# yjhuangcd/rule-guided-music

Hardware: AMD Instinct MI355X
Metric: denoising steps/sec (whole node), DiTRotary_XL_8 4x128x16 (higher is better)
Workload: dtype f32 via bf16x3_presplit split (3 bf16 MFMA per product, fp32 accumulate); 1 GPU; C2 unconditional DDIM-50 (eta=1), DiTRotary_XL_8, batch 16 per GPU, latent 4x128x16; batch_per_gpu=16, weights=synthetic random-init (rgm.synth seed 1; adaLN/final layers re-randomised), timing=one timed region of 255 steps

## Files before the change

### include/rgm.h

```cpp
#ifndef RGM_H
#define RGM_H

#include <stddef.h>
#include <stdint.h>

#ifdef __cplusplus
extern "C" {
#endif

typedef enum {
  RGM_OK = 0,
  RGM_ERR_INVALID = -1,
  RGM_ERR_HIP = -2,
  RGM_ERR_WORKSPACE = -3,
  RGM_ERR_STATE = -4
} rgm_status;

int rgm_version(void);
const char* rgm_last_error(void);

typedef struct rgm_dit rgm_dit;

typedef struct {
  int32_t depth;
  int32_t hidden;
  int32_t heads;
  int32_t patch;
  int32_t in_ch;
  int32_t out_ch;
  int32_t width;
  int32_t n_embed;
  int32_t kind;
  int32_t n_out;
  int32_t max_tokens;
} rgm_dit_cfg;

int rgm_dit_create(const rgm_dit_cfg* cfg, rgm_dit** out);
void rgm_dit_destroy(rgm_dit* h);
int rgm_dit_set_param(rgm_dit* h, const char* key, const void* dptr, const int64_t* shape, int ndim);
int rgm_dit_missing_params(rgm_dit* h);
size_t rgm_dit_workspace_bytes(const rgm_dit* h, int N, int H);
int rgm_dit_forward(rgm_dit* h, const float* x, const int64_t* t, const int32_t* y, float* eps,
                    int N, int H, void* ws, size_t ws_bytes, void* stream);
int rgm_dit_cond_rows(rgm_dit* h, const int64_t* t, const int32_t* y, int U, int H, float* rows, void* ws, size_t ws_bytes, void* stream);
int rgm_dit_forward_cond(rgm_dit* h, const float* x, const float* rows, const int32_t* idx, int U, float* eps,
                         int N, int H, void* ws, size_t ws_bytes, void* stream);
int rgm_dit_classify(rgm_dit* h, const float* x, const int64_t* t, float* logits, float* key_out,
                     int N, int H, void* ws, size_t ws_bytes, void* stream);

int rgm_gemm(const float* A, int lda, const float* B, int ldb, float* C, int ldc, int M, int N, int K,
             const float* bias, int act, float alpha, const float* gate, int gate_ld, int rows_per_gate,
             const float* res, int ldres, void* stream);
int rgm_layernorm_modulate(const float* x, float* out, int M, int D, float eps, const float* weight,
                           const float* bias, const float* shift, const float* scale, int mod_ld,
                           int rows_per_batch, void* stream);
int rgm_adaln_stream(const float* cs, const float* W, const float* bias, float* mod, int N, int D, int L, void* stream);
int rgm_rotary_attention(const float* qkv, float* o, const float* cos_tab, const float* sin_tab,
                         int N, int T, int heads, int hd, int rot_half, void* stream);
int rgm_rotary_attention_lse(const float* qkv, float* o, float* lse, const float* cos_tab, const float* sin_tab,
                             int N, int T, int heads, int hd, int rot_half, void* stream);

int rgm_set_gemm_precision(int prec);
int rgm_get_gemm_precision(void);
int rgm_split_dtype(void);
int rgm_split_rows(const float* x, float* out, int64_t rows, int K, void* stream);
int rgm_gemm_split(const float* A_split, const float* B_split, float* C, int M, int N, int K, const float* bias,
                   int act, int tile, int out_split, void* stream);
int rgm_split_rows_ld(const float* x, int ld_in, float* out, int ld_out, int64_t rows, int K, void* stream);
int rgm_gemm_split_ld(const float* A_split, int lda, const float* B_split, int ldb, float* C, int ldc, int M, int N, int K,
                      const float* bias, int act, int tile, int out_split, void* stream);
int rgm_set_big_tiles(int mode, int min_tiles);
int rgm_set_fuse_reduce_ln(int on);
long long rgm_fused_reduce_ln_launches(void);
int rgm_set_adaln_overlap(int on);
int rgm_set_gn_fuse(int mode, int* prev);
long long rgm_gn_fused_launches(void);
long long rgm_gn_fallback_tiles(int reset);
int rgm_set_dit_halves(int min_batch, int* prev);
int rgm_set_attn_pairs(int on);
int rgm_set_attn_stream(int on);
size_t rgm_gemm_scratch_bytes(int M, int N);
int rgm_gemm_split_ws(const float* A_split, const float* B_split, float* C, int M, int N, int K, const float* bias, int act,
                      int tile, int out_split, void* ws, size_t ws_bytes, void* stream);
int rgm_gemm_split_epi(const float* A_split, int lda, const float* B_split, int ldb, float* C, int ldc, int M, int N, int K,
                       const float* bias, int act, float alpha, const float* gate, int gate_ld, int rows_per_gate,
                       const float* res, int ldres, int tile, int out_split, void* ws, size_t ws_bytes, void* stream);
int rgm_gemm_tile(const float* A, int lda, const float* B, int ldb, float* C, int ldc, int M, int N, int K,
                  const float* bias, int act, int tile, void* stream);

int rgm_randn(float* out, int64_t n, uint64_t seed, uint64_t offset, void* stream);
int rgm_ddpm_step(const float* x, const float* eps, const float* grad, const float* noise, const int64_t* t,
                  const float* const* tables_host, int clip_denoised, int t_end, float* sample, float* pred_xstart,
                  float* g_out, int N, int E, void* stream);
int rgm_ddpm_step_learned(const float* x, const float* eps, const float* var_values, const float* min_log_tab,
                          const float* max_log_tab, const float* grad, const float* noise, const int64_t* t,
                          const float* const* tables_host, int clip_denoised, int t_end, float* sample, float* pred_xstart, int N,
                          int E, void* stream);
int rgm_ddpm_step_learned_g(const float* x, const float* eps, const float* var_values, const float* min_log_tab,
                            const float* max_log_tab, const float* grad, const float* noise, const int64_t* t,
                            const float* const* tables_host, int clip_denoised, int t_end, float* sample, float* pred_xstart,
                            float* g_elem, int N, int E, void* stream);
int rgm_ddim_step(const float* x, const float* eps, const float* grad, const float* noise, const int64_t* t,
                  const float* const* tables_host, int clip_denoised, int t_end, float eta, float* sample,
                  float* pred_xstart, float* g_out, int N, int E, void* stream);
int rgm_dpmpp_step(const float* x, const float* eps, const float* grad, const float* x0_prev, const float* noise, const int64_t* t,
                   const float* const* tables_host, const float* const* dpm_tables_host, int num_timesteps, int order,
                   int clip_denoised, int t_end, float* sample, float* pred_xstart, float* g_out, int N, int E, void* stream);
int rgm_ddim_reverse_step(const float* x, const float* eps, const int64_t* t, const float* const* tables_host, int num_timesteps,
                          int clip_denoised, float* sample, float* pred_xstart, int N, int E, void* stream);
int64_t rgm_vb_terms_partials(int N, int E);
int rgm_vb_terms(const float* x_start, const float* x_t, const float* eps, const float* noise, const int64_t* t,
                 const float* const* tables_host, const float* post_logvar_tab, const float* var_values, const float* min_log_tab,
                 const float* max_log_tab, const float* model_mean, const float* model_xstart, int clip_denoised, double* partials,
                 float* vb, float* xstart_mse, float* eps_mse, float* pred_xstart, int N, int E, void* stream);
int rgm_prior_bpd(const float* x_start, float sqrt_alphas_cumprod_T, float log_one_minus_alphas_cumprod_T, double* partials, float* out,
                  int N, int E, void* stream);
int rgm_scg_candidates(const float* mean, const float* g, const float* noise, float* cand, int n, int B, int E,
                       void* stream);
int rgm_xstart_from_eps(const float* x, const float* eps, const int64_t* t, const float* const* tables_host,
                        float out_scale, float* out, int N, int E, void* stream);
int rgm_edit_replace_eps(const float* x, const float* eps, const float* gt, const float* mask, const int64_t* t,
                         const float* const* tables_host, int clip_denoised, float* eps_out, int N, int E, void* stream);
int rgm_scg_select(const float* cand, const float* total_logp, float* out, int64_t* max_ind, int n, int B, int E,
                   void* stream);
int rgm_scg_rebuild(const float* mean, const float* g, const int64_t* max_ind, uint64_t seed, uint64_t base, float* out,
                    int B, int E, int H, int W, int seg_rows, void* stream);
int rgm_scg_rebuild_g(const float* mean, const float* g_elem, const int64_t* max_ind, uint64_t seed, uint64_t base, float* out,
                      int B, int E, int H, int W, int seg_rows, void* stream);

typedef struct rgm_vae rgm_vae;
int rgm_vae_create(rgm_vae** out);
void rgm_vae_destroy(rgm_vae* h);
int rgm_vae_set_param(rgm_vae* h, const char* key, const void* dptr, const int64_t* shape, int ndim);
int rgm_vae_has_param(rgm_vae* h, const char* key);
int rgm_vae_missing_params(rgm_vae* h);
int rgm_vae_encoder_missing_params(rgm_vae* h);
size_t rgm_vae_workspace_bytes(const rgm_vae* h, int M );
int rgm_vae_decode(rgm_vae* h, const float* z, float* out, int M, void* ws, size_t ws_bytes, void* stream);
int rgm_vae_decode_latent(rgm_vae* h, const float* latent, float inv_scale, float* roll, uint8_t* roll_u8,
                          float threshold, int N, int H, void* ws, size_t ws_bytes, void* stream);
int rgm_vae_encode(rgm_vae* h, const float* x, float* moments, int M, void* ws, size_t ws_bytes, void* stream);
int rgm_vae_enable_grad(rgm_vae* h);
size_t rgm_vae_grad_workspace_bytes(const rgm_vae* h, int M );
int rgm_vae_decode_latent_save(rgm_vae* h, const float* latent, float inv_scale, float* roll, int N, int H, void* ws,
                               size_t ws_bytes, void* stream);
int rgm_vae_decode_latent_vjp(rgm_vae* h, const float* d_roll, float inv_scale, float* d_latent, int N, int H, void* ws,
                              size_t ws_bytes, void* stream);
int rgm_quantise_roll(const float* roll, uint8_t* out_u8, int B, int T, float threshold, void* stream);

int rgm_rule_pitch_hist(float* roll, float* out, float* scratch, int N, int C, int T, void* stream);
int rgm_rule_pitch_hist_vag(float* roll, const float* target, float scale, float* hist, float* logp, float* d_roll,
                            float* scratch, int N, int C, int T, void* stream);
int rgm_rule_note_density(float* roll, float* out, int N, int C, int T, int interval, float hscale, void* stream);
int rgm_rule_chord_quantise(float* roll, uint8_t* out, int N, int C, int T, void* stream);
int rgm_rule_chords(const uint8_t* q, int N, int T, int Wc, const double* profile, const int32_t* given_tonic, int analyse_key,
                    int64_t* chords, int32_t* roots, int32_t* key, double* coef, void* ws, size_t ws_bytes, void* stream);
size_t rgm_note_stats_workspace(int N, int T);
int rgm_note_stats(const uint8_t* roll, long long stride_n, long long stride_c, long long stride_p, long long stride_t, int N, int C,
                   int T, int first_column_onsets, int64_t* out_int, double* out_real, void* ws, size_t ws_bytes, void* stream);
int rgm_roll_to_u8(const float* roll, uint8_t* out, int N, int C, int T, void* stream);
size_t rgm_midi_workspace(int N, int T);
int rgm_midi_measure(const uint8_t* roll, long long stride_n, long long stride_c, long long stride_p, long long stride_t, int N, int C,
                     int T, int first_column_onsets, const int32_t* ticks_host, int64_t* counts, void* ws, size_t ws_bytes, void* stream);
int rgm_midi_emit(int N, int T, int program, const int64_t* note_off, const int64_t* cc_off, const int64_t* byte_off, int32_t* notes,
                  long long notes_cap, int32_t* ccs, long long ccs_cap, uint8_t* bytes, long long bytes_cap, void* ws, size_t ws_bytes,
                  void* stream);
size_t rgm_midi_read_workspace(int N, long long total_bytes, int total_tracks);
int rgm_midi_read_scan(const uint8_t* blob, const int64_t* offsets, int N, long long total_bytes, int total_tracks, double fs, int32_t* status,
                       int64_t* counts, int64_t* columns, int64_t* note_off, int64_t* cc_off, int64_t* notes, long long notes_cap, int64_t* ccs,
                       long long ccs_cap, void* ws, size_t ws_bytes, void* stream);
int rgm_midi_read_rolls(int N, long long total_bytes, int total_tracks, double fs, long long start_column, int T, int out_u8, void* out,
                        int64_t* overflow, void* ws, size_t ws_bytes, void* stream);
int rgm_roll_augment_capacity(int S);
int rgm_roll_augment(const uint8_t* blob, long long blob_bytes, const int64_t* offsets, const int32_t* lengths, int N, const int32_t* params,
                     int B, int S, float* out, int32_t* status, void* stream);
int rgm_latent_windows_count(int n_tiles, int shift_size);
int rgm_latent_windows(const float* moments, int B, int n_tiles, int shift_size, float scale_factor, float* z0, const int64_t* t,
                       const float* sqrt_ac, const float* sqrt_1mac, int num_timesteps, const float* noise, uint64_t seed, uint64_t offset,
                       float* x_t, void* stream);
size_t rgm_latent_std_workspace(long long n);
int rgm_latent_std(const float* x, long long n, double* out, void* ws, size_t ws_bytes, void* stream);
int rgm_set_distances(const double* a, int Na, const double* b, int Nb, int d, int skip_diagonal, double* out, void* stream);
size_t rgm_kde_pdf_workspace(int n, int m);
int rgm_kde_pdf(const double* data, int n, const double* x, int m, double* pdf, void* ws, size_t ws_bytes, void* stream);
size_t rgm_set_kl_oa_workspace(int nA, int nB, int kl_points, int oa_panels);
int rgm_set_kl_oa(const double* A, int nA, const double* B, int nB, int kl_points, int oa_panels, double* out, void* ws, size_t ws_bytes,
                  void* stream);
int rgm_bucketize(const float* v, const float* bounds, int nb, int64_t* out, int n, void* stream);
int rgm_row_loss(const float* a, const float* b, float* out, int rows, int K, int zero_one, void* stream);

size_t rgm_dit_grad_workspace_bytes(const rgm_dit* h, int N, int H);
int rgm_dit_cls_value_and_grad(rgm_dit* h, const float* x, const int64_t* t, const void* target, int loss_kind,
                               float scale, float* logits_out, float* grad_x, int N, int H, void* ws,
                               size_t ws_bytes, void* stream);
int rgm_dit_enable_grad(rgm_dit* h);
int rgm_dit_vjp(rgm_dit* h, const float* x, const int64_t* t, const int32_t* y, const float* g_eps, float* eps_out,
                float* grad_x, int N, int H, void* ws, size_t ws_bytes, void* stream);
int rgm_set_attn_split(int mode);
int rgm_set_attn_bwd_stream(int on);
long long rgm_attn_bwd_stream_launches(void);
int rgm_rotary_attention_bwd(const float* qkv, const float* o, const float* d_o, const float* lse, float* dqkv,
                             const float* cos_tab, const float* sin_tab, int N, int T, int heads, int hd,
                             int rot_half, void* stream);

int rgm_prof_enable(int on);
int rgm_prof_reset(void);
int rgm_prof_report(int kernel, int* launches, double* total_ms, double* total_flops);
double rgm_prof_bytes(int kernel);
int rgm_prof_dump(int cap, int* ids, double* ms, double* flops);
int rgm_gemm2_dbg(int mode, long long* out64);
int rgm_gemm144_dbg(int mode, long long* out64);

int rgm_collage_split(const float* img, float* wins, float* halves, int B, int C, int h, int W, int n, int overlap,
                      void* stream);
int rgm_collage_merge(const float* full, const float* half, float* out, int B, int C, int h, int n, int overlap,
                      int circle, int is_avg, void* stream);

int rgm_particle_resample(const float* reward, double* logw, float* r_prev, double lambda, double ess_frac, const double* u,
                          uint64_t seed, uint64_t counter, int32_t* anc, double* ess_out, int32_t* resampled, int n, int B, void* stream);
int rgm_gather_rows(const float* src, float* dst, const int32_t* anc, int n, int B, int E, void* stream);

#ifdef __cplusplus
}
#endif
#endif
```

### rule-guided-music_amd/csrc/gemm144.hip

```cpp
#include "common.h"

namespace rgm {
void gemm2_prof_set_bytes(int idx, double bytes);
namespace {

typedef split_t bf16x8 __attribute__((ext_vector_type(8)));
typedef float f32x4 __attribute__((ext_vector_type(4)));
#ifdef RGM_SPLIT_F16
#define RGM_MFMA_SPLIT_16x16x32 __builtin_amdgcn_mfma_f32_16x16x32_f16
#else
#define RGM_MFMA_SPLIT_16x16x32 __builtin_amdgcn_mfma_f32_16x16x32_bf16
#endif

__device__ __forceinline__ void dma16(const void* gsrc, void* lds_dst) {
  __builtin_amdgcn_global_load_lds((const __attribute__((address_space(1))) void*)gsrc,
                                   (__attribute__((address_space(3))) void*)lds_dst, 16, 0, 0);
}

constexpr int BM = 128, BN = 144, PAD = 16;
constexpr int ROWS = BM + BN + PAD;
constexpr int STAGE = ROWS * 128;
constexpr int LSEG = ROWS / 8 / 4;
constexpr int TM = 2, TN = 9;

template <int NSTAGE, int DBG = 0, int EXP = 0, int PF = 0>
__global__ __launch_bounds__(512) void gemm144_kernel(GemmParams p, const char* __restrict__ zero_page, int tiles_m, int tiles_n,
                                                      long long* __restrict__ dbg = nullptr, int pf_a = 1) {
  extern __shared__ __attribute__((aligned(16))) char ring[];
  unsigned long long tacc[8] = {0, 0, 0, 0, 0, 0, 0, 0}, t_entry = 0;
  auto now = [&]() {
    const unsigned long long t = __builtin_amdgcn_s_memtime();
    asm volatile("s_waitcnt lgkmcnt(0)" ::: "memory");
    return t;
  };
  unsigned long long rt_entry = 0;
  if (DBG) {
    t_entry = now();
    rt_entry = __builtin_amdgcn_s_memrealtime();
  }
  const int z = blockIdx.z;
  const int bid = blockIdx.x, nb = tiles_m * tiles_n;
  const int xcd = bid & 7, loc = bid >> 3, q = nb >> 3, r = nb & 7;
  const int sid = (xcd < r ? xcd * (q + 1) : r * (q + 1) + (xcd - r) * q) + loc;
  const int G = p.raster_group > 0 ? p.raster_group : tiles_m;
  const int per_group = G * tiles_n, grp = sid / per_group, first_m = grp * G;
  const int gsz = min(tiles_m - first_m, G), in_g = sid - grp * per_group;
  const int m0 = (first_m + in_g % gsz) * BM, n0 = (in_g / gsz) * BN;
  const int tid = threadIdx.x;
  const int wave = __builtin_amdgcn_readfirstlane(tid >> 6);
  const int lane = tid & 63;
  const int KT = p.K >> 5;
  const char* Ab = reinterpret_cast<const char*>(p.A + (long long)z * p.sA);
  const char* Bb = reinterpret_cast<const char*>(p.B + (long long)z * p.sB);

  if (wave >= 4) {
    const int lw = wave - 4, r8 = lane >> 3;
    const char* src[LSEG];
    int inc[LSEG];
#pragma unroll
    for (int i = 0; i < LSEG; ++i) {
      const int row_l = (lw + i * 4) * 8 + r8;
      const int cs = ((lane & 7) ^ ((row_l >> 1) & 7)) << 4;
      const bool isA = row_l < BM;
      const int row = isA ? m0 + row_l : n0 + row_l - BM;
      const bool ok = isA ? row < p.M : (row_l < BM + BN && row < p.N);
      src[i] = ok ? (isA ? Ab + (long long)row * p.lda * 4 : Bb + (long long)row * p.ldb * 4) + cs : zero_page + cs;
      inc[i] = ok ? 128 : 0;
    }
    auto issue_tile = [&](char* dst) {
      static_for<0, LSEG>([&](auto ic) {
        constexpr int i = decltype(ic)::value;
        dma16(src[i], dst + (lw + i * 4) * 1024);
        src[i] += inc[i];
      });
    };
    auto wait_flying = [&](int tiles) {
      static_for<0, NSTAGE - 1>([&](auto c) {
        if (tiles == decltype(c)::value) asm volatile("s_waitcnt vmcnt(%0)" ::"n"(decltype(c)::value * LSEG) : "memory");
      });
    };
    if (DBG) tacc[3] = now() - t_entry;
    static_for<0, NSTAGE - 1>([&](auto c) {
      if (decltype(c)::value < KT) issue_tile(ring + decltype(c)::value * STAGE);
    });
    wait_flying(min(NSTAGE - 2, KT - 1));
    if (DBG) tacc[6] = now() - t_entry;
    __builtin_amdgcn_s_barrier();
    int s2 = NSTAGE - 1;
    unsigned long long t0 = 0;
    if (DBG) {
      t0 = now();
      tacc[2] = t0 - t_entry;
    }
    for (int kt = 0; kt + 1 < KT; ++kt) {
      unsigned long long ta = 0, tb = 0, tc = 0;
      if (DBG) ta = now();
      if (kt + NSTAGE - 1 < KT && !(EXP & 4)) issue_tile(ring + s2 * STAGE);
      if (DBG) tb = now();
      wait_flying(min(NSTAGE - 2, KT - 2 - kt));
      if (DBG) tc = now();
      if constexpr (!(EXP & 1)) __builtin_amdgcn_s_barrier();
      if (DBG) {
        tacc[4] += tb - ta;
        tacc[5] += tc - tb;
        tacc[0] += now() - tc;
      }
      s2 = s2 == NSTAGE - 1 ? 0 : s2 + 1;
    }
    if (DBG) {
      tacc[1] = now() - t0;
      tacc[7] = KT;
      if (blockIdx.x == gridDim.x / 2 && blockIdx.z == 0 && lane == 0)
        for (int i = 0; i < 8; ++i) dbg[wave * 8 + i] = (long long)tacc[i];
    }
    return;
  }

  const int l15 = lane & 15, kb = lane >> 4;
  const int rq = (l15 >> 1) & 7;
  const int arow0 = wave * 32;
  f32x4 acc[TM][TN];
#pragma unroll
  for (int i = 0; i < TM; ++i)
#pragma unroll
    for (int j = 0; j < TN; ++j) acc[i][j] = f32x4{0.f, 0.f, 0.f, 0.f};
  const char* pf_src = zero_page;
  int pf_inc = 0, pf_left = 0;
  char* pf_dst = ring + NSTAGE * STAGE + wave * 256;
  if constexpr (PF > 0) {
    const int q8 = nb >> 3;
    const bool aligned = r == 0 && q8 % gsz == 0 && (per_group % q8 == 0 || q8 % per_group == 0);
    int nA = aligned ? min(q8 / gsz, tiles_n) : 1;
    nA = nA >= 8 ? 8 : nA >= 4 ? 4 : nA >= 2 ? 2 : 1;
    const int nB = aligned ? gsz : 1;
    const int iA = (in_g / gsz) % nA, iB = in_g % gsz % nB;
    const int a_cnt = (nA > 1 && pf_a) ? BM / nA : 0, b_cnt = (BN + nB - 1) / nB;
    const int slot = wave * 64 + lane;
    if (slot < a_cnt) {
      const int row = m0 + iA * a_cnt + slot;
      if (row < p.M) { pf_src = Ab + (long long)row * p.lda * 4; pf_inc = 128; }
    } else if (slot < a_cnt + b_cnt) {
      const int rl = iB * b_cnt + slot - a_cnt, row = n0 + rl;
      if (rl < BN && row < p.N) { pf_src = Bb + (long long)row * p.ldb * 4; pf_inc = 128; }
    }
    pf_src += (long long)pf_inc * (NSTAGE - 1);
    pf_left = KT - (NSTAGE - 1);
    for (int i = NSTAGE - 1; i < PF; ++i) {
      if (pf_left > 0) {
        __builtin_amdgcn_global_load_lds((const __attribute__((address_space(1))) void*)pf_src, (__attribute__((address_space(3))) void*)pf_dst, 4, 0, 0);
        pf_src += pf_inc;
      }
      --pf_left;
    }
  }
  auto prefetch_issue = [&]() {
    if constexpr (PF > 0) {
      if (pf_left > 0)
        __builtin_amdgcn_global_load_lds((const __attribute__((address_space(1))) void*)pf_src, (__attribute__((address_space(3))) void*)pf_dst, 4, 0, 0);
    }
  };
  auto prefetch_advance = [&]() {
    if constexpr (PF > 0) {
      pf_src += pf_inc;
      --pf_left;
    }
  };
  struct Half {
    bf16x8 a[TM], b[TN];
  };
  constexpr int NT = TM * TN;
  auto rd = [&](bf16x8& dst, const char* st, int row, int lo) {
    dst = *reinterpret_cast<const bf16x8*>(st + row * 128 + (((4 * lo + kb) ^ rq) << 4));
  };
  const int ar = arow0 + l15, br = BM + l15;
  auto term = [&](auto tc, const Half& hi, Half& lo, Half& nhi, const char* nst, auto prec) {
    constexpr int T = decltype(tc)::value;
    constexpr bool PRE = decltype(prec)::value != 0;
    static_for<0, NT>([&](auto mc) {
      constexpr int m = decltype(mc)::value;
      constexpr int im = m / TN, in = m % TN;
      if constexpr (T == 0) acc[im][in] = RGM_MFMA_SPLIT_16x16x32(hi.b[in], lo.a[im], acc[im][in], 0, 0, 0);
      if constexpr (T == 1) acc[im][in] = RGM_MFMA_SPLIT_16x16x32(lo.b[in], hi.a[im], acc[im][in], 0, 0, 0);
      if constexpr (T == 2) acc[im][in] = RGM_MFMA_SPLIT_16x16x32(hi.b[in], hi.a[im], acc[im][in], 0, 0, 0);
      if constexpr (PRE && T == 1 && !(EXP & 2)) {
        if constexpr (m < TM) rd(lo.a[m], nst, ar + m * 16, 1);
        else if constexpr (m < 2 * TM) rd(nhi.a[m - TM], nst, ar + (m - TM) * 16, 0);
        else if constexpr (m < 2 * TM + TN) rd(nhi.b[m - 2 * TM], nst, br + (m - 2 * TM) * 16, 0);
      }
      if constexpr (PRE && T == 2 && !(EXP & 2)) {
        if constexpr (m < TN) rd(lo.b[m], nst, br + m * 16, 1);
      }
      if constexpr (PRE && T == 2 && m == TN + 2) prefetch_issue();
      if constexpr (PRE && T == 2 && m == TN + 5) prefetch_advance();
      __builtin_amdgcn_sched_barrier(0);
    });
  };
  using I0 = std::integral_constant<int, 0>;
  using I1 = std::integral_constant<int, 1>;
  using I2 = std::integral_constant<int, 2>;
  static_assert(2 * TM + TN <= NT && TN <= NT, "the next tile's reads fit between the MFMAs of terms 1 and 2");
  Half h0, h1, lo;
  if (DBG) tacc[4] = now() - t_entry;
  __builtin_amdgcn_s_barrier();
  if (DBG) tacc[5] = now() - t_entry;
#pragma unroll
  for (int i = 0; i < TM; ++i) {
    rd(h0.a[i], ring, ar + i * 16, 0);
    rd(lo.a[i], ring, ar + i * 16, 1);
  }
#pragma unroll
  for (int i = 0; i < TN; ++i) {
    rd(h0.b[i], ring, br + i * 16, 0);
    rd(lo.b[i], ring, br + i * 16, 1);
  }
  int s1 = 1;
  auto iter_more = [&](Half& cur, Half& nxt) {
    term(I0{}, cur, lo, nxt, nullptr, I0{});
    asm volatile("s_waitcnt lgkmcnt(0)" ::: "memory");
    unsigned long long ta = 0;
    if (DBG) ta = now();
    if constexpr (!(EXP & 1)) __builtin_amdgcn_s_barrier();
    if (DBG) tacc[0] += now() - ta;
    __builtin_amdgcn_sched_barrier(0);
    const char* nst = ring + s1 * STAGE;
    term(I1{}, cur, lo, nxt, nst, I1{});
    term(I2{}, cur, lo, nxt, nst, I1{});
    s1 = s1 == NSTAGE - 1 ? 0 : s1 + 1;
  };
  auto iter_last = [&](Half& cur) {
    term(I0{}, cur, lo, cur, nullptr, I0{});
    term(I1{}, cur, lo, cur, nullptr, I0{});
    term(I2{}, cur, lo, cur, nullptr, I0{});
  };
  unsigned long long t_loop = 0;
  if (DBG) {
    t_loop = now();
    tacc[2] = t_loop - t_entry;
  }
  int kt = 0;
  for (; kt + 2 < KT; kt += 2) {
    iter_more(h0, h1);
    iter_more(h1, h0);
  }
  if (KT - kt == 2) {
    iter_more(h0, h1);
    iter_last(h1);
  } else {
    iter_last(h0);
  }
  if (DBG) {
    const unsigned long long t = now();
    tacc[1] = t - t_loop;
    t_loop = t;
  }

  float* __restrict__ Cb = p.C + (long long)z * p.sC;
  const float* resb = p.res ? p.res + (long long)z * p.sRes : nullptr;
  const float* biasb = p.bias ? p.bias + (long long)z * p.sBias : nullptr;
  const int colb = n0 + 4 * kb;
  float4 bv[TN];
#pragma unroll
  for (int in = 0; in < TN; ++in) bv[in] = biasb ? *reinterpret_cast<const float4*>(biasb + colb + in * 16) : make_float4(0.f, 0.f, 0.f, 0.f);
  typedef split_t bf16x4 __attribute__((ext_vector_type(4)));
#pragma unroll
  for (int im = 0; im < TM; ++im) {
    const int row = m0 + arow0 + im * 16 + l15;
    const bool ok = row < p.M;
    float4 g4[TN], r4[TN];
    const bool reads = (p.gate || resb) && ok;
    if (reads) {
      const float* gp = p.gate ? p.gate + (long long)(row / p.rows_per_gate) * p.gate_ld + colb : nullptr;
      const float* rp = resb ? resb + (long long)row * p.ldres + colb : nullptr;
#pragma unroll
      for (int in = 0; in < TN; ++in) {
        g4[in] = gp ? *reinterpret_cast<const float4*>(gp + in * 16) : make_float4(1.f, 1.f, 1.f, 1.f);
        r4[in] = rp ? *reinterpret_cast<const float4*>(rp + in * 16) : make_float4(0.f, 0.f, 0.f, 0.f);
      }
    }
#pragma unroll
    for (int in = 0; in < TN; ++in) {
      const int col = colb + in * 16;
      float v[4] = {acc[im][in][0] * p.alpha + bv[in].x, acc[im][in][1] * p.alpha + bv[in].y, acc[im][in][2] * p.alpha + bv[in].z,
                    acc[im][in][3] * p.alpha + bv[in].w};
      if (p.act == 1) {
#pragma unroll
        for (int e = 0; e < 4; ++e) v[e] = silu_f(v[e]);
      } else if (p.act == 2) {
#pragma unroll
        for (int e = 0; e < 4; ++e) v[e] = gelu_tanh_fast_f(v[e]);
      }
      if (reads) {
        v[0] = v[0] * g4[in].x + r4[in].x; v[1] = v[1] * g4[in].y + r4[in].y;
        v[2] = v[2] * g4[in].z + r4[in].z; v[3] = v[3] * g4[in].w + r4[in].w;
      }
      if (p.out_split) {
        bf16x4 hi, lo;
#pragma unroll
        for (int e = 0; e < 4; ++e) {
          hi[e] = (split_t)v[e];
          lo[e] = (split_t)(v[e] - (float)hi[e]);
        }
        split_t* rowp = reinterpret_cast<split_t*>(Cb + (long long)row * p.ldc);
        if (ok) store_split4_maybe_pair<16>(rowp, col, hi, lo);
        continue;
      }
      if (!ok) continue;
      {
        *reinterpret_cast<float4*>(Cb + (long long)row * p.ldc + col) = make_float4(v[0], v[1], v[2], v[3]);
      }
    }
  }
  if (DBG) {
    asm volatile("s_waitcnt vmcnt(0)" ::: "memory");
    tacc[3] = now() - t_loop;
    tacc[7] = KT;
    if (blockIdx.x == gridDim.x / 2 && blockIdx.z == 0 && lane == 0)
      for (int i = 0; i < 8; ++i) dbg[wave * 8 + i] = (long long)tacc[i];
    if (wave == 0 && lane == 0 && blockIdx.z == 0 && blockIdx.x < 4096) {
      long long* w = dbg + 64 + 8 * blockIdx.x;
      const unsigned long long rt = __builtin_amdgcn_s_memrealtime();
      asm volatile("s_waitcnt lgkmcnt(0)" ::: "memory");
      w[0] = (long long)t_entry; w[1] = (long long)now(); w[2] = (long long)rt_entry; w[3] = (long long)rt;
      w[4] = (long long)tacc[1]; w[5] = (long long)tacc[3]; w[6] = (long long)tacc[2]; w[7] = bid;
    }
  }
}

constexpr size_t DBG_SLOTS = 64 + 8 * 4096;
char* g_zero144 = nullptr;
long long* g_dbg144 = nullptr;
}

bool gemm144_supports(const GemmParams& p) {
  if (p.aload || p.stats || p.act >= 3 || p.aux || p.C2 || p.N % BN != 0 || p.K % 32 != 0 || p.K < 64) return false;
  if (((p.N | p.ldc | p.ldres | p.gate_ld) & 3) != 0) return false;
  const uintptr_t al = (uintptr_t)p.C | (uintptr_t)p.res | (uintptr_t)p.bias | (uintptr_t)p.gate;
  if ((al & 15) != 0 || ((p.sC | p.sRes | p.sBias) & 3) != 0) return false;
  if (p.gate && p.rows_per_gate <= 0) return false;
  return true;
}

int gemm144_launch(const GemmParams& p, hipStream_t s) {
  RGM_REQUIRE(gemm144_supports(p), "gemm144: unsupported call (N=%d must be a multiple of 144; dense operands; act 0-2)", p.N);
  if (!g_zero144) {
    RGM_CHECK_HIP(hipMalloc(&g_zero144, 4096));
    RGM_CHECK_HIP(hipMemset(g_zero144, 0, 4096));
  }
  constexpr int NSTAGE = 4;
  constexpr int PFD = 8;
  static const int pf_on = getenv("RGM_G144_PF") ? atoi(getenv("RGM_G144_PF")) : 3;
  const int tm = cdiv(p.M, BM), tn = p.N / BN;
  const size_t lds = (size_t)NSTAGE * STAGE + 1024;
  GemmParams pr = p;
  if (pr.raster_group <= 0) {
    static const int fixed = getenv("RGM_G144_RASTER") ? atoi(getenv("RGM_G144_RASTER")) : 0;
    pr.raster_group = fixed > 0 ? (fixed < tm ? fixed : tm) : (tm < 8 ? tm : 8);
  }
  auto k = pf_on ? gemm144_kernel<NSTAGE, 0, 0, PFD> : gemm144_kernel<NSTAGE>;
  static bool attr = false;
  if (!attr) {
    RGM_CHECK_HIP(hipFuncSetAttribute(reinterpret_cast<const void*>(gemm144_kernel<NSTAGE, 0, 0, PFD>), hipFuncAttributeMaxDynamicSharedMemorySize, (int)lds));
    RGM_CHECK_HIP(hipFuncSetAttribute(reinterpret_cast<const void*>(gemm144_kernel<NSTAGE>), hipFuncAttributeMaxDynamicSharedMemorySize, (int)lds));
    attr = true;
  }
  if (g_dbg144) {
    static const int exp = getenv("RGM_G144_EXP") ? atoi(getenv("RGM_G144_EXP")) : 0;
    auto launch_dbg = [&](auto kd) {
      (void)hipFuncSetAttribute(reinterpret_cast<const void*>(kd), hipFuncAttributeMaxDynamicSharedMemorySize, (int)lds);
      hipLaunchKernelGGL(kd, dim3((unsigned)(tm * tn), 1, (unsigned)p.batch), dim3(512), lds, s, pr, (const char*)g_zero144, tm, tn, g_dbg144, pf_on >> 1);
    };
    switch (exp) {
      case 1: launch_dbg(gemm144_kernel<NSTAGE, 1, 1, PFD>); break;
      case 2: launch_dbg(gemm144_kernel<NSTAGE, 1, 2, PFD>); break;
      case 4: launch_dbg(gemm144_kernel<NSTAGE, 1, 4, PFD>); break;
      case 7: launch_dbg(gemm144_kernel<NSTAGE, 1, 7, PFD>); break;
      default:
        if (pf_on) launch_dbg(gemm144_kernel<NSTAGE, 1, 0, PFD>);
        else launch_dbg(gemm144_kernel<NSTAGE, 1, 0>);
    }
    RGM_LAUNCH_CHECK();
    return RGM_OK;
  }
  const int pi = gemm2_prof_begin(135, 2.0 * p.M * (double)p.N * p.K * p.batch, s);
  gemm2_prof_set_bytes(pi, 4.0 * ((double)p.M * p.K * p.batch + (double)p.N * p.K * p.batch + (double)p.M * p.N * p.batch * (p.res ? 2.0 : 1.0)));
  hipLaunchKernelGGL(k, dim3((unsigned)(tm * tn), 1, (unsigned)p.batch), dim3(512), lds, s, pr, (const char*)g_zero144, tm, tn, (long long*)nullptr, pf_on >> 1);
  gemm2_prof_end(pi, s);
  RGM_LAUNCH_CHECK();
  return RGM_OK;
}
}

extern "C" int rgm_gemm144_dbg(int mode, long long* out64) {
  using namespace rgm;
  if (mode == 1) {
    if (!g_dbg144) RGM_CHECK_HIP(hipMalloc(&g_dbg144, DBG_SLOTS * sizeof(long long)));
    RGM_CHECK_HIP(hipMemset(g_dbg144, 0, DBG_SLOTS * sizeof(long long)));
  } else if (mode == 2 || mode == 3) {
    RGM_REQUIRE(g_dbg144 && out64, "gemm144_dbg: not armed");
    RGM_CHECK_HIP(hipDeviceSynchronize());
    RGM_CHECK_HIP(hipMemcpy(out64, g_dbg144, (mode == 3 ? DBG_SLOTS : 64) * sizeof(long long), hipMemcpyDeviceToHost));
  } else {
    if (g_dbg144) (void)hipFree(g_dbg144);
    g_dbg144 = nullptr;
  }
  return RGM_OK;
}
```

### rule-guided-music_amd/rgm/native.py

```python
import ctypes as C
import os

_HERE = os.path.dirname(os.path.abspath(__file__))
LIB_PATH = os.environ.get("RGM_LIB_PATH", os.path.join(_HERE, "librgm_hip.so"))


class RgmError(RuntimeError):
    pass


class DitCfg(C.Structure):
    _fields_ = [(n, C.c_int32) for n in ("depth", "hidden", "heads", "patch", "in_ch", "out_ch", "width",
                                         "n_embed", "kind", "n_out", "max_tokens")]


def _load():
    if not os.path.exists(LIB_PATH):
        raise RgmError(f"{LIB_PATH} is missing: build it with `python -c 'import __graft_entry__ as g; g.build()'` "
                       "(or `make -C rule-guided-music_amd/csrc`).  There is no CPU fallback.")
    L = C.CDLL(LIB_PATH)
    vp, i32, f32, sz = C.c_void_p, C.c_int, C.c_float, C.c_size_t
    sig = {
        "rgm_version": (C.c_int, []),
        "rgm_last_error": (C.c_char_p, []),
        "rgm_dit_create": (C.c_int, [C.POINTER(DitCfg), C.POINTER(vp)]),
        "rgm_dit_destroy": (None, [vp]),
        "rgm_dit_set_param": (C.c_int, [vp, C.c_char_p, vp, C.POINTER(C.c_int64), i32]),
        "rgm_dit_missing_params": (C.c_int, [vp]),
        "rgm_dit_workspace_bytes": (sz, [vp, i32, i32]),
        "rgm_dit_forward": (C.c_int, [vp, vp, vp, vp, vp, i32, i32, vp, sz, vp]),
        "rgm_dit_cond_rows": (C.c_int, [vp, vp, vp, i32, i32, vp, vp, sz, vp]),
        "rgm_dit_forward_cond": (C.c_int, [vp, vp, vp, vp, i32, vp, i32, i32, vp, sz, vp]),
        "rgm_dit_classify": (C.c_int, [vp, vp, vp, vp, vp, i32, i32, vp, sz, vp]),
        "rgm_gemm": (C.c_int, [vp, i32, vp, i32, vp, i32, i32, i32, i32, vp, i32, f32, vp, i32, i32, vp, i32, vp]),
        "rgm_gemm_tile": (C.c_int, [vp, i32, vp, i32, vp, i32, i32, i32, i32, vp, i32, i32, vp]),
        "rgm_adaln_stream": (C.c_int, [vp, vp, vp, vp, i32, i32, i32, vp]),
        "rgm_layernorm_modulate": (C.c_int, [vp, vp, i32, i32, f32, vp, vp, vp, vp, i32, i32, vp]),
        "rgm_rotary_attention": (C.c_int, [vp, vp, vp, vp, i32, i32, i32, i32, i32, vp]),
        "rgm_rotary_attention_lse": (C.c_int, [vp, vp, vp, vp, vp, i32, i32, i32, i32, i32, vp]),
        "rgm_randn": (C.c_int, [vp, C.c_int64, C.c_uint64, C.c_uint64, vp]),
        "rgm_ddpm_step": (C.c_int, [vp, vp, vp, vp, vp, vp, i32, i32, vp, vp, vp, i32, i32, vp]),
        "rgm_ddpm_step_learned": (C.c_int, [vp, vp, vp, vp, vp, vp, vp, vp, vp, i32, i32, vp, vp, i32, i32, vp]),
        "rgm_ddpm_step_learned_g": (C.c_int, [vp, vp, vp, vp, vp, vp, vp, vp, vp, i32, i32, vp, vp, vp, i32, i32, vp]),
        "rgm_scg_rebuild_g": (C.c_int, [vp, vp, vp, C.c_uint64, C.c_uint64, vp, i32, i32, i32, i32, i32, vp]),
        "rgm_ddim_step": (C.c_int, [vp, vp, vp, vp, vp, vp, i32, i32, f32, vp, vp, vp, i32, i32, vp]),
        "rgm_dpmpp_step": (C.c_int, [vp, vp, vp, vp, vp, vp, vp, vp, i32, i32, i32, i32, vp, vp, vp, i32, i32, vp]),
        "rgm_ddim_reverse_step": (C.c_int, [vp, vp, vp, vp, i32, i32, vp, vp, i32, i32, vp]),
        "rgm_vb_terms_partials": (C.c_int64, [i32, i32]),
        "rgm_vb_terms": (C.c_int, [vp] * 12 + [i32, vp, vp, vp, vp, vp, i32, i32, vp]),
        "rgm_prior_bpd": (C.c_int, [vp, f32, f32, vp, vp, i32, i32, vp]),
        "rgm_scg_candidates": (C.c_int, [vp, vp, vp, vp, i32, i32, i32, vp]),
        "rgm_xstart_from_eps": (C.c_int, [vp, vp, vp, vp, f32, vp, i32, i32, vp]),
        "rgm_edit_replace_eps": (C.c_int, [vp, vp, vp, vp, vp, vp, i32, vp, i32, i32, vp]),
        "rgm_scg_select": (C.c_int, [vp, vp, vp, vp, i32, i32, i32, vp]),
        "rgm_scg_rebuild": (C.c_int, [vp, vp, vp, C.c_uint64, C.c_uint64, vp, i32, i32, i32, i32, i32, vp]),
        "rgm_vae_create": (C.c_int, [C.POINTER(vp)]),
        "rgm_vae_destroy": (None, [vp]),
        "rgm_vae_set_param": (C.c_int, [vp, C.c_char_p, vp, C.POINTER(C.c_int64), i32]),
        "rgm_vae_has_param": (C.c_int, [vp, C.c_char_p]),
        "rgm_vae_missing_params": (C.c_int, [vp]),
        "rgm_vae_encoder_missing_params": (C.c_int, [vp]),
        "rgm_vae_encode": (C.c_int, [vp, vp, vp, i32, vp, sz, vp]),
        "rgm_vae_workspace_bytes": (sz, [vp, i32]),
        "rgm_vae_decode": (C.c_int, [vp, vp, vp, i32, vp, sz, vp]),
        "rgm_vae_decode_latent": (C.c_int, [vp, vp, f32, vp, vp, f32, i32, i32, vp, sz, vp]),
        "rgm_vae_enable_grad": (C.c_int, [vp]),
        "rgm_vae_grad_workspace_bytes": (sz, [vp, i32]),
        "rgm_vae_decode_latent_save": (C.c_int, [vp, vp, f32, vp, i32, i32, vp, sz, vp]),
        "rgm_vae_decode_latent_vjp": (C.c_int, [vp, vp, f32, vp, i32, i32, vp, sz, vp]),
        "rgm_quantise_roll": (C.c_int, [vp, vp, i32, i32, f32, vp]),
        "rgm_rule_pitch_hist": (C.c_int, [vp, vp, vp, i32, i32, i32, vp]),
        "rgm_rule_pitch_hist_vag": (C.c_int, [vp, vp, f32, vp, vp, vp, vp, i32, i32, i32, vp]),
        "rgm_rule_note_density": (C.c_int, [vp, vp, i32, i32, i32, i32, f32, vp]),
        "rgm_rule_chord_quantise": (C.c_int, [vp, vp, i32, i32, i32, vp]),
        "rgm_rule_chords": (C.c_int, [vp, i32, i32, i32, vp, vp, i32, vp, vp, vp, vp, vp, sz, vp]),
        "rgm_note_stats_workspace": (sz, [i32, i32]),
        "rgm_note_stats": (C.c_int, [vp] + [C.c_longlong] * 4 + [i32, i32, i32, i32, vp, vp, vp, sz, vp]),
        "rgm_roll_to_u8": (C.c_int, [vp, vp, i32, i32, i32, vp]),
        "rgm_midi_workspace": (sz, [i32, i32]),
        "rgm_midi_measure": (C.c_int, [vp] + [C.c_longlong] * 4 + [i32, i32, i32, i32, vp, vp, vp, sz, vp]),
        "rgm_midi_emit": (C.c_int, [i32, i32, i32, vp, vp, vp, vp, C.c_longlong, vp, C.c_longlong, vp, C.c_longlong, vp, sz, vp]),
        "rgm_midi_read_workspace": (sz, [i32, C.c_longlong, i32]),
        "rgm_midi_read_scan": (C.c_int, [vp, vp, i32, C.c_longlong, i32, C.c_double, vp, vp, vp, vp, vp, vp, C.c_longlong, vp, C.c_longlong, vp, sz, vp]),
        "rgm_midi_read_rolls": (C.c_int, [i32, C.c_longlong, i32, C.c_double, C.c_longlong, i32, i32, vp, vp, vp, sz, vp]),
        "rgm_roll_augment_capacity": (C.c_int, [i32]),
        "rgm_roll_augment": (C.c_int, [vp, C.c_longlong, vp, vp, i32, vp, i32, i32, vp, vp, vp]),
        "rgm_latent_windows_count": (C.c_int, [i32, i32]),
        "rgm_latent_windows": (C.c_int, [vp, i32, i32, i32, f32, vp, vp, vp, vp, i32, vp, C.c_uint64, C.c_uint64, vp, vp]),
        "rgm_latent_std_workspace": (sz, [C.c_longlong]),
        "rgm_latent_std": (C.c_int, [vp, C.c_longlong, vp, vp, sz, vp]),
        "rgm_set_distances": (C.c_int, [vp, i32, vp, i32, i32, i32, vp, vp]),
        "rgm_kde_pdf_workspace": (sz, [i32, i32]),
        "rgm_kde_pdf": (C.c_int, [vp, i32, vp, i32, vp, vp, sz, vp]),
        "rgm_set_kl_oa_workspace": (sz, [i32, i32, i32, i32]),
        "rgm_set_kl_oa": (C.c_int, [vp, i32, vp, i32, i32, i32, vp, vp, sz, vp]),
        "rgm_particle_resample": (C.c_int, [vp, vp, vp, C.c_double, C.c_double, vp, C.c_uint64, C.c_uint64, vp, vp, vp, i32, i32, vp]),
        "rgm_gather_rows": (C.c_int, [vp, vp, vp, i32, i32, i32, vp]),
        "rgm_bucketize": (C.c_int, [vp, vp, i32, vp, i32, vp]),
        "rgm_row_loss": (C.c_int, [vp, vp, vp, i32, i32, i32, vp]),
        "rgm_collage_split": (C.c_int, [vp, vp, vp, i32, i32, i32, i32, i32, i32, vp]),
        "rgm_collage_merge": (C.c_int, [vp, vp, vp, i32, i32, i32, i32, i32, i32, i32, vp]),
        "rgm_dit_grad_workspace_bytes": (sz, [vp, i32, i32]),
        "rgm_dit_cls_value_and_grad": (C.c_int, [vp, vp, vp, vp, i32, f32, vp, vp, i32, i32, vp, sz, vp]),
        "rgm_dit_enable_grad": (C.c_int, [vp]),
        "rgm_dit_vjp": (C.c_int, [vp, vp, vp, vp, vp, vp, vp, i32, i32, vp, sz, vp]),
        "rgm_rotary_attention_bwd": (C.c_int, [vp, vp, vp, vp, vp, vp, vp, i32, i32, i32, i32, i32, vp]),
        "rgm_split_rows": (C.c_int, [vp, vp, C.c_int64, i32, vp]),
        "rgm_gemm_split": (C.c_int, [vp, vp, vp, i32, i32, i32, vp, i32, i32, i32, vp]),
        "rgm_gemm_scratch_bytes": (sz, [i32, i32]),
        "rgm_set_big_tiles": (C.c_int, [i32, i32]),
        "rgm_set_fuse_reduce_ln": (C.c_int, [i32]),
        "rgm_set_adaln_overlap": (C.c_int, [i32]),
        "rgm_set_dit_halves": (C.c_int, [i32, vp]),
        "rgm_set_attn_pairs": (C.c_int, [i32]),
        "rgm_set_attn_stream": (C.c_int, [i32]),
        "rgm_set_attn_bwd_stream": (C.c_int, [i32]),
        "rgm_attn_bwd_stream_launches": (C.c_longlong, []),
        "rgm_set_gn_fuse": (C.c_int, [i32, vp]),
        "rgm_gn_fused_launches": (C.c_longlong, []),
        "rgm_gn_fallback_tiles": (C.c_longlong, [i32]),
        "rgm_split_dtype": (C.c_int, []),
        "rgm_set_attn_split": (C.c_int, [i32]),
        "rgm_fused_reduce_ln_launches": (C.c_longlong, []),
        "rgm_gemm_split_ws": (C.c_int, [vp, vp, vp, i32, i32, i32, vp, i32, i32, i32, vp, sz, vp]),
        "rgm_gemm_split_epi": (C.c_int, [vp, i32, vp, i32, vp, i32, i32, i32, i32, vp, i32, f32, vp, i32, i32, vp, i32, i32, i32, vp, sz, vp]),
        "rgm_split_rows_ld": (C.c_int, [vp, i32, vp, i32, C.c_int64, i32, vp]),
        "rgm_gemm_split_ld": (C.c_int, [vp, i32, vp, i32, vp, i32, i32, i32, i32, vp, i32, i32, i32, vp]),
        "rgm_set_gemm_precision": (C.c_int, [i32]),
        "rgm_get_gemm_precision": (C.c_int, []),
        "rgm_prof_enable": (C.c_int, [i32]),
        "rgm_prof_reset": (C.c_int, []),
        "rgm_prof_report": (C.c_int, [i32, C.POINTER(C.c_int), C.POINTER(C.c_double), C.POINTER(C.c_double)]),
        "rgm_prof_bytes": (C.c_double, [i32]),
        "rgm_prof_dump": (C.c_int, [i32, C.POINTER(C.c_int), C.POINTER(C.c_double), C.POINTER(C.c_double)]),
        "rgm_gemm2_dbg": (C.c_int, [i32, C.POINTER(C.c_longlong)]),
        "rgm_gemm144_dbg": (C.c_int, [i32, C.POINTER(C.c_longlong)]),
    }
    for name, (res, args) in sig.items():
        fn = getattr(L, name)
        fn.restype = res
        fn.argtypes = args
    return L


class _Lazy:
    _lib = None

    def __getattr__(self, name):
        if _Lazy._lib is None:
            _Lazy._lib = _load()
        return getattr(_Lazy._lib, name)


lib = _Lazy()
PRECISIONS = {"fp32": 0, "bf16x3": 1, "bf16x3_presplit": 2}


def set_gemm_precision(name):
    check(lib.rgm_set_gemm_precision(PRECISIONS[name]))


class gemm_precision_scope:

    def __init__(self, name):
        self.name = name
        self.prev = None

    def __enter__(self):
        self.prev = int(lib.rgm_get_gemm_precision())
        if self.name is not None:
            check(lib.rgm_set_gemm_precision(PRECISIONS[self.name]))
        return self

    def __exit__(self, *exc):
        check(lib.rgm_set_gemm_precision(self.prev))
        return False


def check(status):
    if status != 0:
        raise RgmError(f"librgm_hip status {status}: {lib.rgm_last_error().decode()}")


def require_cuda(*tensors):
    for t in tensors:
        if t is not None and not t.is_cuda:
            raise RgmError("rgm ops need tensors on a HIP device (no CPU fallback in the product path)")


def ptr(t):
    if t is None:
        return None
    if not t.is_contiguous():
        raise RgmError("rgm ops need contiguous tensors")
    return C.c_void_p(t.data_ptr())


def current_stream():
    import torch
    return C.c_void_p(torch.cuda.current_stream().cuda_stream)
```

Measured before the change: 84.60 steps/s.

## Stage gemm144 epilogue through LDS and prefetch bias/gate/residual during K loop

Adds an EPI variant of the 128x144 GEMM kernel, on by default. The loader waves issue the bias, gate and residual loads during the final K iterations, so those reads overlap the MFMA tail rather than stalling the epilogue. The accumulators are then staged through the LDS ring, and all 8 waves write row-contiguous float4 chunks instead of scattered fragments. This costs extra LDS traffic, two more barriers and more registers for the prefetched operands, which may affect occupancy.

```diff
diff --git a/include/rgm.h b/include/rgm.h
--- a/include/rgm.h
+++ b/include/rgm.h
@@ -77,6 +77,7 @@
 long long rgm_gn_fused_launches(void);
 long long rgm_gn_fallback_tiles(int reset);
 int rgm_set_dit_halves(int min_batch, int* prev);
+int rgm_set_gemm144_epilogue(int mode, int* prev);
 int rgm_set_attn_pairs(int on);
 int rgm_set_attn_stream(int on);
 size_t rgm_gemm_scratch_bytes(int M, int N);
diff --git a/rule-guided-music_amd/csrc/gemm144.hip b/rule-guided-music_amd/csrc/gemm144.hip
--- a/rule-guided-music_amd/csrc/gemm144.hip
+++ b/rule-guided-music_amd/csrc/gemm144.hip
@@ -22,8 +22,30 @@
 constexpr int STAGE = ROWS * 128;
 constexpr int LSEG = ROWS / 8 / 4;
 constexpr int TM = 2, TN = 9;
-
-template <int NSTAGE, int DBG = 0, int EXP = 0, int PF = 0>
+constexpr int CHUNKS = BN / 4;
+constexpr int EROW = BN * 4 + 16;
+constexpr int EITER = BM * CHUNKS / 512;
+constexpr int ELOADS = 3 * EITER;
+static_assert(BM * CHUNKS % 512 == 0 && CHUNKS % 2 == 0 && (64 * EITER) % CHUNKS == 0, "a wave owns whole rows; lane parity is chunk parity");
+
+__device__ __forceinline__ void epi_chunk(float (&v)[4], const f32x4& a, float alpha, const float4& b, int act, bool reads, const float4& g,
+                                          const float4& r) {
+  v[0] = __builtin_fmaf(a[0], alpha, b.x); v[1] = __builtin_fmaf(a[1], alpha, b.y);
+  v[2] = __builtin_fmaf(a[2], alpha, b.z); v[3] = __builtin_fmaf(a[3], alpha, b.w);
+  if (act == 1) {
+#pragma unroll
+    for (int e = 0; e < 4; ++e) v[e] = silu_f(v[e]);
+  } else if (act == 2) {
+#pragma unroll
+    for (int e = 0; e < 4; ++e) v[e] = gelu_tanh_fast_f(v[e]);
+  }
+  if (reads) {
+    v[0] = __builtin_fmaf(v[0], g.x, r.x); v[1] = __builtin_fmaf(v[1], g.y, r.y);
+    v[2] = __builtin_fmaf(v[2], g.z, r.z); v[3] = __builtin_fmaf(v[3], g.w, r.w);
+  }
+}
+
+template <int NSTAGE, int DBG = 0, int EXP = 0, int PF = 0, int EPI = 0>
 __global__ __launch_bounds__(512) void gemm144_kernel(GemmParams p, const char* __restrict__ zero_page, int tiles_m, int tiles_n,
                                                       long long* __restrict__ dbg = nullptr, int pf_a = 1) {
   extern __shared__ __attribute__((aligned(16))) char ring[];
@@ -52,6 +74,39 @@
   const int KT = p.K >> 5;
   const char* Ab = reinterpret_cast<const char*>(p.A + (long long)z * p.sA);
   const char* Bb = reinterpret_cast<const char*>(p.B + (long long)z * p.sB);
+  unsigned long long t_loop = 0;
+  float4 e_b[EITER], e_g[EITER], e_r[EITER];
+  auto epi_request = [&]() {
+    const float* resb = p.res ? p.res + (long long)z * p.sRes : nullptr;
+    const float* biasb = p.bias ? p.bias + (long long)z * p.sBias : nullptr;
+    const int row0 = min(m0 + 16 * wave, p.M - 1);
+    const int rpg = p.gate ? p.rows_per_gate : 1, q0 = row0 / rpg, rem0 = row0 - q0 * rpg;
+    const float rcp = __builtin_amdgcn_rcpf((float)rpg);
+    const float* bp = biasb ? biasb : reinterpret_cast<const float*>(zero_page);
+    const float* gp = p.gate ? p.gate : reinterpret_cast<const float*>(zero_page);
+    const float* rp = resb ? resb : reinterpret_cast<const float*>(zero_page);
+    const int bm = biasb ? 1 : 0, gm = p.gate ? 1 : 0, rm = resb ? 1 : 0;
+    const long long gld = p.gate ? p.gate_ld : 0, rld = resb ? p.ldres : 0;
+    static_for<0, EITER>([&](auto ic) { e_b[decltype(ic)::value] = make_float4(0.f, 0.f, 0.f, 0.f); });
+    if (biasb || p.gate || resb) {
+      static_for<0, EITER>([&](auto ic) {
+        constexpr int it = decltype(ic)::value;
+        const int idx = it * 64 + lane;
+        e_b[it] = ldg16(bp + (n0 + 4 * (idx % CHUNKS)) * bm);
+      });
+    }
+    if (p.gate || resb) {
+      static_for<0, EITER>([&](auto ic) {
+        constexpr int it = decltype(ic)::value;
+        const int idx = it * 64 + lane, col = n0 + 4 * (idx % CHUNKS);
+        const int row = min(m0 + 16 * wave + idx / CHUNKS, p.M - 1), x = rem0 + (row - row0);
+        const int gr = q0 + (rpg >= 16 ? (x >= rpg ? 1 : 0) : (int)(((float)x + 0.5f) * rcp));
+        e_g[it] = ldg16(gp + gr * gld + col * gm);
+        e_r[it] = ldg16(rp + row * rld + col * rm);
+      });
+    }
+  };
+  const int epi_loads = (p.gate || p.res) ? ELOADS : p.bias ? EITER : 0;
 
   if (wave >= 4) {
     const int lw = wave - 4, r8 = lane >> 3;
@@ -74,16 +129,24 @@
         src[i] += inc[i];
       });
     };
-    auto wait_flying = [&](int tiles) {
+    auto wait_flying = [&](int tiles, auto rq) {
       static_for<0, NSTAGE - 1>([&](auto c) {
-        if (tiles == decltype(c)::value) asm volatile("s_waitcnt vmcnt(%0)" ::"n"(decltype(c)::value * LSEG) : "memory");
+        if (tiles == decltype(c)::value) {
+          constexpr int pieces = decltype(c)::value * LSEG;
+          if (decltype(rq)::value && epi_loads == ELOADS) asm volatile("s_waitcnt vmcnt(%0)" ::"n"(pieces + ELOADS) : "memory");
+          else if (decltype(rq)::value && epi_loads == EITER) asm volatile("s_waitcnt vmcnt(%0)" ::"n"(pieces + EITER) : "memory");
+          else asm volatile("s_waitcnt vmcnt(%0)" ::"n"(pieces) : "memory");
+        }
       });
     };
+    using L0 = std::integral_constant<int, 0>;
+    using L1 = std::integral_constant<int, 1>;
+    static_assert((NSTAGE - 2) * LSEG + ELOADS <= 63, "vmcnt has six bits");
     if (DBG) tacc[3] = now() - t_entry;
     static_for<0, NSTAGE - 1>([&](auto c) {
       if (decltype(c)::value < KT) issue_tile(ring + decltype(c)::value * STAGE);
     });
-    wait_flying(min(NSTAGE - 2, KT - 1));
+    wait_flying(min(NSTAGE - 2, KT - 1), L0{});
     if (DBG) tacc[6] = now() - t_entry;
     __builtin_amdgcn_s_barrier();
     int s2 = NSTAGE - 1;
@@ -92,12 +155,12 @@
       t0 = now();
       tacc[2] = t0 - t_entry;
     }
-    for (int kt = 0; kt + 1 < KT; ++kt) {
+    auto loop_tile = [&](int kt, auto issue, auto rq) {
       unsigned long long ta = 0, tb = 0, tc = 0;
       if (DBG) ta = now();
-      if (kt + NSTAGE - 1 < KT && !(EXP & 4)) issue_tile(ring + s2 * STAGE);
+      if (decltype(issue)::value && !(EXP & 4)) issue_tile(ring + s2 * STAGE);
       if (DBG) tb = now();
-      wait_flying(min(NSTAGE - 2, KT - 2 - kt));
+      wait_flying(min(NSTAGE - 2, KT - 2 - kt), rq);
       if (DBG) tc = now();
       if constexpr (!(EXP & 1)) __builtin_amdgcn_s_barrier();
       if (DBG) {
@@ -106,6 +169,14 @@
         tacc[0] += now() - tc;
       }
       s2 = s2 == NSTAGE - 1 ? 0 : s2 + 1;
+    };
+    int kt = 0;
+    for (; kt + NSTAGE - 1 < KT; ++kt) loop_tile(kt, L1{}, L0{});
+    if constexpr (EPI != 0) {
+      epi_request();
+      for (; kt + 1 < KT; ++kt) loop_tile(kt, L0{}, L1{});
+    } else {
+      for (; kt + 1 < KT; ++kt) loop_tile(kt, L0{}, L0{});
     }
     if (DBG) {
       tacc[1] = now() - t0;
@@ -113,9 +184,12 @@
       if (blockIdx.x == gridDim.x / 2 && blockIdx.z == 0 && lane == 0)
         for (int i = 0; i < 8; ++i) dbg[wave * 8 + i] = (long long)tacc[i];
     }
-    return;
-  }
-
+    if constexpr (EPI == 0) return;
+    wait_flying(0, L1{});
+    __builtin_amdgcn_s_barrier();
+    __builtin_amdgcn_s_barrier();
+    asm volatile("" ::: "memory");
+  } else {
   const int l15 = lane & 15, kb = lane >> 4;
   const int rq = (l15 >> 1) & 7;
   const int arow0 = wave * 32;
@@ -232,7 +306,6 @@
     term(I1{}, cur, lo, cur, nullptr, I0{});
     term(I2{}, cur, lo, cur, nullptr, I0{});
   };
-  unsigned long long t_loop = 0;
   if (DBG) {
     t_loop = now();
     tacc[2] = t_loop - t_entry;
@@ -254,6 +327,7 @@
     t_loop = t;
   }
 
+  if constexpr (EPI == 0) {
   float* __restrict__ Cb = p.C + (long long)z * p.sC;
   const float* resb = p.res ? p.res + (long long)z * p.sRes : nullptr;
   const float* biasb = p.bias ? p.bias + (long long)z * p.sBias : nullptr;
@@ -280,19 +354,8 @@
 #pragma unroll
     for (int in = 0; in < TN; ++in) {
       const int col = colb + in * 16;
-      float v[4] = {acc[im][in][0] * p.alpha + bv[in].x, acc[im][in][1] * p.alpha + bv[in].y, acc[im][in][2] * p.alpha + bv[in].z,
-                    acc[im][in][3] * p.alpha + bv[in].w};
-      if (p.act == 1) {
-#pragma unroll
-        for (int e = 0; e < 4; ++e) v[e] = silu_f(v[e]);
-      } else if (p.act == 2) {
-#pragma unroll
-        for (int e = 0; e < 4; ++e) v[e] = gelu_tanh_fast_f(v[e]);
-      }
-      if (reads) {
-        v[0] = v[0] * g4[in].x + r4[in].x; v[1] = v[1] * g4[in].y + r4[in].y;
-        v[2] = v[2] * g4[in].z + r4[in].z; v[3] = v[3] * g4[in].w + r4[in].w;
-      }
+      float v[4];
+      epi_chunk(v, acc[im][in], p.alpha, bv[in], p.act, reads, g4[in], r4[in]);
       if (p.out_split) {
         bf16x4 hi, lo;
 #pragma unroll
@@ -309,6 +372,47 @@
         *reinterpret_cast<float4*>(Cb + (long long)row * p.ldc + col) = make_float4(v[0], v[1], v[2], v[3]);
       }
     }
+  }
+  } else {
+    epi_request();
+    __builtin_amdgcn_s_barrier();
+#pragma unroll
+    for (int im = 0; im < TM; ++im)
+#pragma unroll
+      for (int in = 0; in < TN; ++in)
+        *reinterpret_cast<f32x4*>(ring + (arow0 + im * 16 + l15) * EROW + (in * 16 + 4 * kb) * 4) = acc[im][in];
+    asm volatile("s_waitcnt lgkmcnt(0)" ::: "memory");
+    __builtin_amdgcn_s_barrier();
+    asm volatile("" ::: "memory");
+  }
+  }
+
+  if constexpr (EPI != 0) {
+    typedef split_t bf16x4 __attribute__((ext_vector_type(4)));
+    float* __restrict__ Cb = p.C + (long long)z * p.sC;
+    const bool reads = p.gate || p.res;
+    static_for<0, EITER>([&](auto ic) {
+      constexpr int it = decltype(ic)::value;
+      const int idx = it * 64 + lane, rl = 16 * wave + idx / CHUNKS, ch = idx % CHUNKS;
+      const int row = m0 + rl, col = n0 + 4 * ch;
+      const f32x4 a = *reinterpret_cast<const f32x4*>(ring + rl * EROW + ch * 16);
+      float v[4];
+      epi_chunk(v, a, p.alpha, e_b[it], p.act, reads, p.gate ? e_g[it] : make_float4(1.f, 1.f, 1.f, 1.f), e_r[it]);
+      if (row < p.M) {
+        if (p.out_split) {
+          bf16x4 hi, lo;
+#pragma unroll
+          for (int e = 0; e < 4; ++e) {
+            hi[e] = (split_t)v[e];
+            lo[e] = (split_t)(v[e] - (float)hi[e]);
+          }
+          store_split4_maybe_pair<1>(reinterpret_cast<split_t*>(Cb + (long long)row * p.ldc), col, hi, lo);
+        } else {
+          *reinterpret_cast<float4*>(Cb + (long long)row * p.ldc + col) = make_float4(v[0], v[1], v[2], v[3]);
+        }
+      }
+    });
+    if (wave >= 4) return;
   }
   if (DBG) {
     asm volatile("s_waitcnt vmcnt(0)" ::: "memory");
@@ -329,6 +433,7 @@
 constexpr size_t DBG_SLOTS = 64 + 8 * 4096;
 char* g_zero144 = nullptr;
 long long* g_dbg144 = nullptr;
+int g_epi144 = getenv("RGM_G144_EPI") ? (atoi(getenv("RGM_G144_EPI")) == 0 ? 0 : 1) : 1;
 }
 
 bool gemm144_supports(const GemmParams& p) {
@@ -356,11 +461,15 @@
     static const int fixed = getenv("RGM_G144_RASTER") ? atoi(getenv("RGM_G144_RASTER")) : 0;
     pr.raster_group = fixed > 0 ? (fixed < tm ? fixed : tm) : (tm < 8 ? tm : 8);
   }
-  auto k = pf_on ? gemm144_kernel<NSTAGE, 0, 0, PFD> : gemm144_kernel<NSTAGE>;
+  const int epi = g_epi144;
+  auto k = epi ? (pf_on ? gemm144_kernel<NSTAGE, 0, 0, PFD, 1> : gemm144_kernel<NSTAGE, 0, 0, 0, 1>)
+               : (pf_on ? gemm144_kernel<NSTAGE, 0, 0, PFD> : gemm144_kernel<NSTAGE>);
   static bool attr = false;
   if (!attr) {
     RGM_CHECK_HIP(hipFuncSetAttribute(reinterpret_cast<const void*>(gemm144_kernel<NSTAGE, 0, 0, PFD>), hipFuncAttributeMaxDynamicSharedMemorySize, (int)lds));
     RGM_CHECK_HIP(hipFuncSetAttribute(reinterpret_cast<const void*>(gemm144_kernel<NSTAGE>), hipFuncAttributeMaxDynamicSharedMemorySize, (int)lds));
+    RGM_CHECK_HIP(hipFuncSetAttribute(reinterpret_cast<const void*>(gemm144_kernel<NSTAGE, 0, 0, PFD, 1>), hipFuncAttributeMaxDynamicSharedMemorySize, (int)lds));
+    RGM_CHECK_HIP(hipFuncSetAttribute(reinterpret_cast<const void*>(gemm144_kernel<NSTAGE, 0, 0, 0, 1>), hipFuncAttributeMaxDynamicSharedMemorySize, (int)lds));
     attr = true;
   }
   if (g_dbg144) {
@@ -369,15 +478,20 @@
       (void)hipFuncSetAttribute(reinterpret_cast<const void*>(kd), hipFuncAttributeMaxDynamicSharedMemorySize, (int)lds);
       hipLaunchKernelGGL(kd, dim3((unsigned)(tm * tn), 1, (unsigned)p.batch), dim3(512), lds, s, pr, (const char*)g_zero144, tm, tn, g_dbg144, pf_on >> 1);
     };
-    switch (exp) {
-      case 1: launch_dbg(gemm144_kernel<NSTAGE, 1, 1, PFD>); break;
-      case 2: launch_dbg(gemm144_kernel<NSTAGE, 1, 2, PFD>); break;
-      case 4: launch_dbg(gemm144_kernel<NSTAGE, 1, 4, PFD>); break;
-      case 7: launch_dbg(gemm144_kernel<NSTAGE, 1, 7, PFD>); break;
-      default:
-        if (pf_on) launch_dbg(gemm144_kernel<NSTAGE, 1, 0, PFD>);
-        else launch_dbg(gemm144_kernel<NSTAGE, 1, 0>);
-    }
+    auto launch_exp = [&](auto ec) {
+      constexpr int E = decltype(ec)::value;
+      switch (exp) {
+        case 1: launch_dbg(gemm144_kernel<NSTAGE, 1, 1, PFD, E>); break;
+        case 2: launch_dbg(gemm144_kernel<NSTAGE, 1, 2, PFD, E>); break;
+        case 4: launch_dbg(gemm144_kernel<NSTAGE, 1, 4, PFD, E>); break;
+        case 7: launch_dbg(gemm144_kernel<NSTAGE, 1, 7, PFD, E>); break;
+        default:
+          if (pf_on) launch_dbg(gemm144_kernel<NSTAGE, 1, 0, PFD, E>);
+          else launch_dbg(gemm144_kernel<NSTAGE, 1, 0, 0, E>);
+      }
+    };
+    if (epi) launch_exp(std::integral_constant<int, 1>{});
+    else launch_exp(std::integral_constant<int, 0>{});
     RGM_LAUNCH_CHECK();
     return RGM_OK;
   }
@@ -405,3 +519,10 @@
   }
   return RGM_OK;
 }
+
+extern "C" int rgm_set_gemm144_epilogue(int mode, int* prev) {
+  RGM_REQUIRE(mode == 0 || mode == 1, "set_gemm144_epilogue: %d (0 / 1)", mode);
+  if (prev) *prev = rgm::g_epi144;
+  rgm::g_epi144 = mode;
+  return RGM_OK;
+}
diff --git a/rule-guided-music_amd/rgm/native.py b/rule-guided-music_amd/rgm/native.py
--- a/rule-guided-music_amd/rgm/native.py
+++ b/rule-guided-music_amd/rgm/native.py
@@ -112,6 +112,7 @@
         "rgm_set_fuse_reduce_ln": (C.c_int, [i32]),
         "rgm_set_adaln_overlap": (C.c_int, [i32]),
         "rgm_set_dit_halves": (C.c_int, [i32, vp]),
+        "rgm_set_gemm144_epilogue": (C.c_int, [i32, vp]),
         "rgm_set_attn_pairs": (C.c_int, [i32]),
         "rgm_set_attn_stream": (C.c_int, [i32]),
         "rgm_set_attn_bwd_stream": (C.c_int, [i32]),
```

New measurement: 85.63 steps/s, median of 6. +1.2%, better.
